# WoojuLee24/OA-DG

Hardware: AMD Instinct MI355X
Metric: images/sec training, Faster R-CNN R50-FPN + OA-DG, 1024x2048 (higher is better)
Workload: dtype bf16

## Files before the change

include/oadg_hip.h:

```cpp
#ifndef OADG_HIP_H
#define OADG_HIP_H

#include <stddef.h>
#include <stdint.h>

#ifdef __cplusplus
extern "C" {
#endif

size_t oadg_supcon_workspace_bytes(int B, int D);
int oadg_supcon_fwd(const float* feats, const int64_t* labels, int B, int D, int n_labels, int ori_size,
                    int rp_size, float temper, int min_samples, float loss_weight, void* workspace,
                    size_t workspace_bytes, float* out_loss, void* stream);
int oadg_supcon_bwd(const int64_t* labels, int B, int D, int n_labels, int ori_size, int rp_size,
                    float temper, float loss_weight, const float* grad_out, void* workspace,
                    size_t workspace_bytes, float* dfeats, void* stream);
int oadg_supcon_status(const void* workspace_host_copy);

size_t oadg_cls_loss_workspace_bytes(void);
int oadg_ce_jsd_fwd(const float* logits, const int64_t* labels, const float* weights, long R, int C,
                    int mode, float avg_factor, float loss_weight, float lambda_jsd, void* workspace,
                    size_t workspace_bytes, float* out3, void* stream);
int oadg_ce_jsd_bwd(const float* logits, const int64_t* labels, const float* weights, long R, int C,
                    int mode, float avg_factor, float loss_weight, float lambda_jsd, const float* grad_out,
                    float* dlogits, void* stream);

int oadg_roi_align_fwd(const void* const* feats_host, const int* heights_host, const int* widths_host,
                       const float* scales_host, int levels, int N, int C, int dtype, float finest_scale,
                       const float* rois, int K, int PH, int PW, int sampling_ratio, int aligned,
                       void* out, const int* order, void* stream);
int oadg_roi_align_bwd(float* const* dfeats_host, const int* heights_host, const int* widths_host,
                       const float* scales_host, int levels, int N, int C, int dtype, float finest_scale,
                       const float* rois, int K, int PH, int PW, int sampling_ratio, int aligned,
                       const void* grad_out, const int* order, void* stream);
int oadg_roi_order_keys(const float* rois, int K, int n_img, int levels, float finest_scale, long long* keys,
                        void* stream);
int oadg_roi_order(const float* rois, int K, int n_img, int levels, float finest_scale, int* order, int* range,
                   void* stream);
int oadg_roi_align_bwd_tiles(void* const* dmaps, const int* heights, const int* widths, const float* scales,
                             int levels, int N, int C, float finest_scale, const float* rois, int K, int PH, int PW,
                             int sampling_ratio, int aligned, const void* grad_out, const int* order, const int* range,
                             void* tile_boxes, void* stream);

typedef struct oadg_rpn_loss_level {
    const void* y;
    void* gy;
    long sN, sC, sH, sW;
    int H, W, Cy;
    long first, pix0;
} oadg_rpn_loss_level;
size_t oadg_rpn_loss_workspace_bytes(void);
int oadg_rpn_loss_fwd(const oadg_rpn_loss_level* levels, int n_levels, int B, int A, long At, int dtype,
                      const int64_t* labels, const float* label_weights, const float* bbox_targets,
                      const float* bbox_weights, float avg_factor, float w_cls, float lambda_jsd, float w_box,
                      void* workspace, size_t workspace_bytes, float* out4, void* stream);
int oadg_rpn_loss_bwd(const oadg_rpn_loss_level* levels, int n_levels, int B, int A, long At, int dtype,
                      const int64_t* labels, const float* label_weights, const float* bbox_targets,
                      const float* bbox_weights, float avg_factor, float w_cls, float lambda_jsd, float w_box,
                      const float* grad_cls, const float* grad_box, void* stream);

#define OADG_RPN_MAX_LEVELS 8
typedef struct oadg_rpn_level {
    const void* deltas;
    long sN, sC, sH, sW;
    const float* anchors;
    const float* scores;
    const long long* index;
    int H, W, A, k, dtype, first;
} oadg_rpn_level;
int oadg_rpn_decode(const oadg_rpn_level* levels, int n_levels, int n_img, const float* means4, const float* stds4,
                    float max_ratio, const float* lim, int clip, float min_size, float* props, float* scores,
                    unsigned char* valid, void* stream);
int oadg_rpn_order(const oadg_rpn_level* levels, int n_levels, int n_img, const float* props, const float* scores,
                   const unsigned char* valid, float* boxes_sorted, int* order, int* counts, float* max_coord,
                   void* stream);
// ... 212 lines not shown

int oadg_conv2d_nhwc_bf16_scatter(const void* x, const void* w, const float* bias, const void* residual, void* y,
                                  const void* zeros16, int N, int H, int W, int C, int K, int R, int S, int pad, int dil,
                                  int relu, int out_h, int out_w, int OH, int OW, int osh, int osw, int oph, int opw,
                                  const void* mask, float* colsum_part, const void* mask_bits, void* stream);
int oadg_conv2d_dgrad_s2_nhwc_bf16(const void* dy, const void* wt, const void* residual, void* dx, const void* zeros16,
                                   int N, int Ho, int Wo, int K, int C, int R, int H, int W, const void* mask,
                                   float* colsum_part, const void* mask_bits, void* stream);

int oadg_prep_conv_weights(const float* w, const float* gamma, const float* beta, const float* mean,
                           const float* var, float eps, const float* bias_in, int K, int C, int R, int S, void* wf,
                           void* wt, float* bias, float* scale, int w_krsc, int wt_mode, void* stream);
typedef struct oadg_prep_desc {
    const float *w, *gamma, *beta, *mean, *var, *bias_in;
    void *wf, *wt;
    float *bias, *scale;
    float eps;
    int K, C, R, S, w_krsc, wt_mode, first_block;
} oadg_prep_desc;
int oadg_prep_conv_weights_multi_blocks(int K, int C, int R, int S);
int oadg_prep_conv_weights_multi(const oadg_prep_desc* descs, int n_layers, int total_blocks, void* stream);
int oadg_prep_conv_weights_bwd(const void* gwf, const float* gbias, const float* w, const float* scale,
                               const float* mean, const float* var, float eps, int K, int C, int R, int S, float* dw,
                               float* dgamma, int w_krsc, void* stream);

int oadg_conv1x1_n16_fwd(const void* x, const void* w16, const float* bias16, void* y, long M, int C, void* stream);
long oadg_conv1x1_n16_dgrad_rows(long M);
int oadg_conv1x1_n16_dgrad(const void* dy, const void* wt, void* dx, const void* mask_bits, float* colsum_part, long M, int C,
                           void* stream);
long oadg_conv1x1_n16_wgrad_splits(long M);
long oadg_conv1x1_n16_wgrad_rows(long M);
int oadg_conv1x1_n16_wgrad(const void* x, const void* dy, float* part, float* bias_part, const void* zeros16, long M, int C,
                           void* stream);

int oadg_stem_conv7x7s2_nhwc_bf16(const void* x, const void* wp, void* y, int N, int H, int W, void* stream);

int oadg_bias_relu_maxpool_nhwc_bf16(const void* x, const float* bias, void* out, int N, int H, int W, int C,
                                     void* stream);

size_t oadg_relu_bias_bwd_workspace_bytes(long M, int K);
int oadg_relu_bias_bwd(const void* dy, int dy_is_f32, const void* y, void* g, float* dbias, void* workspace,
                       size_t workspace_bytes, long M, int K, void* stream);

int oadg_fpn_topdown_fwd(const void* lat, const void* top, void* out, int N, int H, int W, int Ht, int Wt, int C,
                         void* stream);
int oadg_fpn_topdown_bwd(const void* g, void* dtop, int N, int H, int W, int Ht, int Wt, int C, void* stream);

size_t oadg_max_iou_assign_workspace_bytes(int B, int Gmax);
int oadg_max_iou_assign(const float* boxes, long box_stride, const unsigned char* valid, const float* gts,
                        const int* gt_counts, const int64_t* gt_labels, int B, int N, int Gmax, float pos_iou_thr,
                        float neg_iou_lo, float neg_iou_hi, float min_pos_iou, int match_low_quality,
                        void* workspace, size_t workspace_bytes, int64_t* gt_inds, float* max_overlaps,
                        int64_t* labels, int* counts, void* stream);

typedef struct oadg_select_job {
    const void* gt_inds;
    long n;
    int mode;
    int k;
    int all;
    int rank_off;
    long out_off;
} oadg_select_job;
size_t oadg_sample_select_workspace_bytes(int jobs, long max_n);
int oadg_sample_select(const oadg_select_job* jobs_dev, int jobs, long max_n, int max_k, const int* ranks_dev,
                       int64_t* out, void* workspace, size_t workspace_bytes, void* stream);
// ... 104 lines not shown
```

oa-dg_amd/_lib.py:

```python
import ctypes
import os
from ctypes import (POINTER, Structure, c_char_p, c_double, c_float, c_int, c_int32, c_int64, c_long, c_longlong, c_size_t,
                    c_uint16, c_void_p)

import numpy as np

_HERE = os.path.dirname(os.path.abspath(__file__))
LIB_PATH = os.environ.get('OADG_HIP_LIB') or os.path.join(_HERE, 'csrc', 'liboadg_hip.so')
_lib = None

vp, ci, cf, cl, cs, cd = c_void_p, c_int, c_float, c_long, c_size_t, c_double


class RpnLevel(Structure):
    _fields_ = [('deltas', c_void_p), ('sN', c_long), ('sC', c_long), ('sH', c_long), ('sW', c_long), ('anchors', c_void_p),
                ('scores', c_void_p), ('index', c_void_p), ('H', c_int), ('W', c_int), ('A', c_int), ('k', c_int),
                ('dtype', c_int), ('first', c_int)]


class RpnLossLevel(Structure):
    _fields_ = [('y', c_void_p), ('gy', c_void_p), ('sN', c_long), ('sC', c_long), ('sH', c_long), ('sW', c_long),
                ('H', c_int), ('W', c_int), ('Cy', c_int), ('first', c_long), ('pix0', c_long)]


class RoiAssignImage(Structure):
    _fields_ = [('proposals', c_void_p), ('gt_bboxes', c_void_p), ('gt_labels', c_void_p), ('stride', c_int),
                ('num_gts', c_int)]


ROI_ASSIGN_MAX_IMAGES = 32


class RoiTargetEntry(Structure):
    _fields_ = [('bboxes', c_void_p), ('gt_bboxes', c_void_p), ('gt_inds', c_void_p), ('labels', c_void_p),
                ('pos_inds', c_void_p), ('neg_inds', c_void_p), ('npos', c_int), ('nneg', c_int), ('stride', c_int),
                ('batch', c_int)]


ROI_TARGET_MAX_ENTRIES = 32


class RoiSampleImage(Structure):
    _fields_ = [('gt_inds', c_void_p), ('n', c_int)]


ROI_SAMPLE_MAX_IMAGES = 8
RPN_MAX_LEVELS = 8
PARSE_LOSSES_MAX = 32


class RegionOp(Structure):
    _fields_ = [('kind', c_int), ('param', c_int), ('image', c_void_p), ('minv', c_double * 6)]


OP_COPY, OP_LUT_AUTOCONTRAST, OP_LUT_EQUALIZE, OP_POSTERIZE, OP_SOLARIZE, OP_IMAGE, OP_BG_WARP, OP_WARP_NEG = range(8)
# ... 25 lines not shown
        _f(ci, 'K C R S w_krsc wt_mode first_block')


class SelectJob(Structure):
    _fields_ = [('gt_inds', vp), ('n', cl)] + _f(ci, 'mode k all rank_off') + [('out_off', cl)]


class SgdTensor(Structure):
    _fields_ = _f(vp, 'param grad momentum') + _f(c_longlong, 'numel first_block') + _f(ci, 'first_step pad')


class MixTarget(Structure):
    _fields_ = [('fg_index', ci), ('rect', ci * 4), ('m_oa', cf)]


class BboxStep(Structure):
    _fields_ = [('minv', cd * 6), ('rect', ci * 4), ('row', ci), ('pad_', ci), ('scratch_off', c_longlong)]


class BboxChain(Structure):
    _fields_ = _f(vp, 'img steps_dev tile_prefix_dev level_first_host tile_prefix_host My Mx scratch') + \
        _f(ci, 'H W n_levels pad_')


class JpegDesc(Structure):
    _fields_ = _f(c_int32, 'height width ncomp hmax vmax mcux mcuy reserved') + _f(c_int32 * 4, 'h v bw bh cw ch') + \
        [('off', c_int64 * 4), ('qt', c_uint16 * 64 * 4)]


COLSUM_JOB, WGRAD_JOB, PREP_BWD_JOB, PREP_DESC, SELECT_JOB, SGD_TENSOR, MIX_TARGET, BBOX_STEP, BBOX_CHAIN = (
    np.dtype(c) for c in (ColsumJob, WgradJob, PrepBwdJob, PrepDesc, SelectJob, SgdTensor, MixTarget, BboxStep, BboxChain))

STRUCTS = {
    'oadg_rpn_level': RpnLevel, 'oadg_rpn_loss_level': RpnLossLevel, 'oadg_roi_assign_image': RoiAssignImage,
    'oadg_roi_target_entry': RoiTargetEntry, 'oadg_roi_sample_image': RoiSampleImage, 'oadg_region_op': RegionOp,
    'oadg_colsum_job': ColsumJob, 'oadg_wgrad_job': WgradJob, 'oadg_prep_bwd_job': PrepBwdJob, 'oadg_prep_desc': PrepDesc,
    'oadg_select_job': SelectJob, 'oadg_sgd_tensor': SgdTensor, 'oadg_mix_target': MixTarget, 'oadg_bbox_step': BboxStep,
    'oadg_bbox_chain': BboxChain, 'oadg_jpeg_desc': JpegDesc,
}

SIGNATURES = {
    'oadg_supcon_workspace_bytes': (cs, [ci, ci]),
    'oadg_supcon_fwd': (ci, [vp, vp, ci, ci, ci, ci, ci, cf, ci, cf, vp, cs, vp, vp]),
    'oadg_supcon_bwd': (ci, [vp, ci, ci, ci, ci, ci, cf, cf, vp, vp, cs, vp, vp]),
    'oadg_supcon_status': (ci, [vp]),
    'oadg_cls_loss_workspace_bytes': (cs, []),
    'oadg_ce_jsd_fwd': (ci, [vp, vp, vp, cl, ci, ci, cf, cf, cf, vp, cs, vp, vp]),
    'oadg_ce_jsd_bwd': (ci, [vp, vp, vp, cl, ci, ci, cf, cf, cf, vp, vp, vp]),
    'oadg_roi_align_fwd': (ci, [POINTER(vp), POINTER(ci), POINTER(ci), POINTER(cf), ci, ci, ci, ci, cf,
                                vp, ci, ci, ci, ci, ci, vp, vp, vp]),
    'oadg_roi_align_bwd': (ci, [POINTER(vp), POINTER(ci), POINTER(ci), POINTER(cf), ci, ci, ci, ci, cf,
                                vp, ci, ci, ci, ci, ci, vp, vp, vp]),
    'oadg_roi_order_keys': (ci, [vp, ci, ci, ci, cf, vp, vp]),
    'oadg_roi_order': (ci, [vp, ci, ci, ci, cf, vp, vp, vp]),
    'oadg_roi_align_bwd_tiles': (ci, [POINTER(vp), POINTER(ci), POINTER(ci), POINTER(cf), ci, ci, ci, cf, vp, ci, ci, ci,
                                      ci, ci, vp, vp, vp, vp, vp]),
    'oadg_rpn_loss_workspace_bytes': (cs, []),
    'oadg_rpn_loss_fwd': (ci, [vp, ci, ci, ci, cl, ci, vp, vp, vp, vp, cf, cf, cf, cf, vp, cs, vp, vp]),
    'oadg_rpn_loss_bwd': (ci, [vp, ci, ci, ci, cl, ci, vp, vp, vp, vp, cf, cf, cf, cf, vp, vp, vp]),
    'oadg_rpn_decode': (ci, [vp, ci, ci, vp, vp, cf, vp, ci, cf, vp, vp, vp, vp]),
    'oadg_rpn_order': (ci, [vp, ci, ci, vp, vp, vp, vp, vp, vp, vp, vp]),
    'oadg_rpn_gather': (ci, [ci, ci, ci, vp, vp, vp, vp, vp, vp, vp]),
    'oadg_rpn_topk_workspace_bytes': (cs, [POINTER(ci), ci, ci, ci]),
    'oadg_rpn_topk': (ci, [POINTER(vp), POINTER(cl), POINTER(ci), ci, ci, ci, ci, POINTER(vp), POINTER(vp), vp, cs, vp]),
    'oadg_nms_workspace_bytes': (cs, [ci, ci]),
    'oadg_nms_batched': (ci, [vp, vp, ci, ci, cf, ci, vp, cs, vp, vp, vp]),
    'oadg_resize_bilinear_u8': (ci, [vp, ci, ci, ci, vp, ci, ci, vp]),
    'oadg_flip_u8': (ci, [vp, ci, ci, ci, vp, ci, vp]),
    'oadg_conv2d_nhwc_bf16': (ci, [vp, vp, vp, vp, vp, vp] + [ci] * 11 + [vp]),
    'oadg_conv2d_auto_variant': (ci, [ci] * 10),
    'oadg_conv2d_nhwc_bf16_ex': (ci, [vp, vp, vp, vp, vp, vp] + [ci] * 12 + [vp, vp, vp, vp, vp]),
    'oadg_conv2d_pixel_tiles': (cl, [ci] * 11),
    'oadg_colsum_reduce': (ci, [vp, cl, ci, vp, vp]),
    'oadg_conv2d_nhwc_bf16_variant': (ci, [vp, vp, vp, vp, vp, vp] + [ci] * 12 + [vp]),
    'oadg_conv2d_wgrad_workspace_bytes': (cs, [ci] * 7),
    'oadg_conv2d_wgrad_variant': (ci, [ci] * 7),
    'oadg_conv2d_wgrad_nhwc_bf16': (ci, [vp, vp, vp, vp, vp, cs] + [ci] * 10 + [vp]),
    'oadg_conv2d_wgrad_parts_nhwc_bf16': (ci, [vp, vp, vp, vp, cs] + [ci] * 10 + [POINTER(ci), vp]),
    'oadg_prep_conv_weights_bwd_parts': (ci, [vp, ci, vp, vp, vp, vp, vp, cf, ci, ci, ci, ci, vp, vp, ci, vp]),
    'oadg_prep_conv_weights': (ci, [vp, vp, vp, vp, vp, cf, vp, ci, ci, ci, ci, vp, vp, vp, vp, ci, ci, vp]),
    'oadg_prep_conv_weights_multi': (ci, [vp, ci, ci, vp]),
    'oadg_prep_conv_weights_multi_blocks': (ci, [ci, ci, ci, ci]),
    'oadg_conv2d_nhwc_bf16_scatter': (ci, [vp, vp, vp, vp, vp, vp] + [ci] * 18 + [vp, vp, vp, vp]),
    'oadg_conv2d_dgrad_s2_nhwc_bf16': (ci, [vp, vp, vp, vp, vp, ci, ci, ci, ci, ci, ci, ci, ci, vp, vp, vp, vp]),
    'oadg_prep_conv_weights_bwd': (ci, [vp, vp, vp, vp, vp, vp, cf, ci, ci, ci, ci, vp, vp, ci, vp]),
    'oadg_relu_bias_bwd_workspace_bytes': (ctypes.c_size_t, [cl, ci]),
    'oadg_relu_bias_bwd': (ci, [vp, ci, vp, vp, vp, vp, ctypes.c_size_t, cl, ci, vp]),
    'oadg_stem_conv7x7s2_nhwc_bf16': (ci, [vp, vp, vp, ci, ci, ci, vp]),
    'oadg_bias_relu_maxpool_nhwc_bf16': (ci, [vp, vp, vp, ci, ci, ci, ci, vp]),
    'oadg_fpn_topdown_fwd': (ci, [vp, vp, vp, ci, ci, ci, ci, ci, ci, vp]),
    'oadg_fpn_topdown_bwd': (ci, [vp, vp, ci, ci, ci, ci, ci, ci, vp]),
    'oadg_max_iou_assign_workspace_bytes': (ctypes.c_size_t, [ci, ci]),
    'oadg_max_iou_assign': (ci, [vp, cl, vp, vp, vp, vp, ci, ci, ci, cf, cf, cf, cf, ci, vp, ctypes.c_size_t, vp, vp, vp,
                                 vp, vp]),
    'oadg_sample_select_workspace_bytes': (ctypes.c_size_t, [ci, cl]),
    'oadg_sample_select': (ci, [vp, ci, cl, ci, vp, vp, vp, ctypes.c_size_t, vp]),
    'oadg_anchor_targets': (ci, [vp, vp, vp, vp, vp, vp, ci, ci, ci, ci, c_int64, cf, vp, vp, vp, vp, vp, vp, vp]),
    'oadg_colsum_reduce_multi': (ci, [vp, ci, ci, vp]),
    'oadg_conv1x1_n16_fwd': (ci, [vp, vp, vp, vp, cl, ci, vp]),
    'oadg_conv1x1_n16_dgrad_rows': (cl, [cl]),
    'oadg_conv1x1_n16_dgrad': (ci, [vp, vp, vp, vp, vp, cl, ci, vp]),
    'oadg_bottleneck_frozen_256': (ci, [vp, vp, vp, vp, vp, vp, vp, vp, ci, ci, ci, vp]),
    'oadg_bottleneck_frozen_first_64': (ci, [vp, vp, vp, vp, vp, vp, vp, vp, vp, vp, ci, ci, ci, vp]),
    'oadg_conv1x1_n16_wgrad_splits': (cl, [cl]),
    'oadg_conv1x1_n16_wgrad_rows': (cl, [cl]),
    'oadg_conv1x1_n16_wgrad': (ci, [vp, vp, vp, vp, vp, cl, ci, vp]),
    'oadg_conv2d_wgrad_multi_plan': (ctypes.c_long, [vp, ci, ci, vp]),
    'oadg_conv2d_wgrad_multi': (ci, [vp, ci, ci, vp, vp, vp]),
    'oadg_prep_conv_weights_bwd_parts_multi': (ci, [vp, ci, ci, ci, vp]),
    'oadg_sgd_blocks': (ctypes.c_longlong, [ctypes.c_longlong]),
    'oadg_sgd_step_multi': (ci, [vp, ci, ctypes.c_longlong, cf, cf, cf, vp]),
    'oadg_fc_weight_permute': (ci, [vp, vp, ci, ci, ci, ci, vp]),
    'oadg_parse_losses': (ci, [vp, vp, ci, ci, ctypes.c_uint, vp, vp, vp]),
    'oadg_roi_reg_acc_fwd': (ci, [vp, ci, vp, ci, vp, vp, vp, ci, ci, ci, ci, ci, cf, cf, cf, vp, vp]),
    'oadg_roi_reg_bwd': (ci, [vp, ci, vp, vp, vp, ci, ci, ci, ci, cf, cf, cf, vp, vp, vp]),
    'oadg_roi_assign_add_gt': (ci, [vp, ci, ci, ci, cf, cf, cf, cf, ci, vp, vp, vp, vp, vp, vp, vp, vp, vp, ctypes.c_size_t,
                                    vp, vp]),
    'oadg_roi_targets': (ci, [vp, ci, ci, c_int64, cf, vp, vp, vp, vp, vp, vp, vp, vp, vp]),
    'oadg_roi_targets_dev': (ci, [vp, ci, ci, ci, vp, c_int64, cf, vp, vp, vp, vp, vp, vp, vp, vp, vp]),
    'oadg_roi_sample_max_rows': (ci, []),
    'oadg_roi_sample_device': (ci, [vp, ci, ci, ci, cd, vp, vp, vp, vp, vp, vp]),
    'oadg_conv2d_f32': (ci, [vp, vp, vp, vp, vp, ci, ci, ci, ci, ci, ci, ci, ci, ci, ci, ci, ci, ci, vp]),
    'oadg_conv2d_wgrad_f32_splits': (ci, [ci, ci, ci, ci, ci, ci, ci]),
    'oadg_conv2d_wgrad_f32': (ci, [vp, vp, vp, vp, cs, ci, ci, ci, ci, ci, ci, ci, ci, ci, ci, vp]),
    'oadg_host_randperm_prefix': (ci, [vp, POINTER(ci), POINTER(ctypes.c_uint64), c_int64, c_int64, vp]),
    'oadg_np_random_bboxes': (ci, [vp, ci, ci, ci, vp, ci, cd, cd, cd, cd, ci, cd, cd, vp]),
    'oadg_oamix_box_profiles': (ci, [vp, vp, ci, ci, ci, ci, vp, vp, vp]),
    'oadg_oamix_fg_union': (ci, [vp, vp, ci, ci, ci, vp, vp, vp]),
    'oadg_oamix_fg_union_rects': (ci, [vp, vp, vp, ci, ci, ci, vp, vp, vp]),
    'oadg_oamix_saliency_workspace_bytes': (cs, [ci]),
    'oadg_oamix_saliency': (ci, [vp, ci, ci, vp, ci, ci, vp, vp, cs, vp]),
    'oadg_oamix_saliency_batch': (ci, [vp, ctypes.c_longlong, vp, ci, ci, vp, ci, ci, vp, vp, ctypes.c_size_t, vp]),
    'oadg_oamix_hist': (ci, [vp, cl, vp, vp]),
    'oadg_oamix_luts': (ci, [vp, vp, vp]),
    'oadg_oamix_gray_sum': (ci, [vp, cl, vp, vp]),
    'oadg_oamix_bbox_step': (ci, [vp, ci, ci, POINTER(cd), ci, ci, ci, ci, vp, vp, vp, vp]),
    'oadg_oamix_bbox_levels': (ci, [POINTER(ci), POINTER(cd), ci, ci, ci, POINTER(ci)]),
    'oadg_oamix_bbox_plan_bytes': (cs, [ci]),
    'oadg_oamix_bbox_plan': (ci, [ci, cd, vp, vp, ci, vp, ci, ci, ci, vp, cs, vp, vp, vp]),
# ... 72 lines not shown
```

oa-dg_amd/csrc/narrow_head.hip:

```cpp
#include "common.h"
#include "oadg_hip.h"

namespace {

typedef float f32x4n __attribute__((ext_vector_type(4)));
typedef short v4sn __attribute__((ext_vector_type(4)));
typedef __attribute__((address_space(3))) v4sn* lds_v4sn_ptr;
typedef __attribute__((address_space(3))) void* lds_ptr_n;
typedef const __attribute__((address_space(1))) void* gbl_ptr_n;

__device__ __forceinline__ void glds16n(const void* g, void* l) {
    __builtin_amdgcn_global_load_lds((gbl_ptr_n)g, (lds_ptr_n)l, 16, 0, 0);
}

#define ZERO8 (bf16x8{0, 0, 0, 0, 0, 0, 0, 0})

__device__ __forceinline__ int kofs(int ks, int fq) { return 64 * (ks >> 1) + 16 * fq + 8 * (ks & 1); }

template <int C>
__global__ __launch_bounds__(256) void n16_fwd_kernel(const unsigned short* __restrict__ x,
                                                      const unsigned short* __restrict__ w16,
                                                      const float* __restrict__ bias16, unsigned short* __restrict__ y,
                                                      long M) {
    constexpr int KS = C / 32;
// ... 286 lines not shown
    const long splits = n16_splits(M), nchunks = (M + NWP - 1) / NWP;
    const int cps = (int)((nchunks + splits - 1) / splits);
    const unsigned grid = (unsigned)((nchunks + cps - 1) / cps);
    if ((long)grid != splits && (long)grid > splits) return OADG_EARG;
    hipStream_t st = (hipStream_t)stream;
#define OADG_N16W(CC)                                                                                                     \
    do {                                                                                                                  \
        constexpr int LDS = 2 * (NWP * CC * 2 + NWP * 32);                                                                \
        static bool attr = false;                                                                                         \
        if (!attr) {                                                                                                      \
            hipError_t e = hipFuncSetAttribute((const void*)n16_wgrad_kernel<CC>,                                         \
                                               hipFuncAttributeMaxDynamicSharedMemorySize, LDS);                          \
            if (e != hipSuccess) return (int)e;                                                                           \
            attr = true;                                                                                                  \
        }                                                                                                                 \
        hipLaunchKernelGGL(n16_wgrad_kernel<CC>, dim3(grid), dim3(256), LDS, st, (const unsigned short*)x,                \
                           (const unsigned short*)dy, part, bias_part, (const unsigned short*)zeros16, M, cps);           \
    } while (0)
    if (C == 256) OADG_N16W(256);
    else if (C == 128) OADG_N16W(128);
    else return OADG_EARG;
#undef OADG_N16W
    OADG_LAUNCH_CHECK();
    return OADG_OK;
}

long oadg_conv1x1_n16_wgrad_rows(long M) {
    if (M < 1) return 0;
    const long splits = n16_splits(M), nchunks = (M + NWP - 1) / NWP;
    const long cps = (nchunks + splits - 1) / splits;
    return (nchunks + cps - 1) / cps;
}

}
```

oa-dg_amd/csrc/roi_align.hip:

```cpp
#include "common.h"
#include <stdlib.h>

#define OADG_MAX_LEVELS 8

namespace {

struct Pyramid {
    const void* feat[OADG_MAX_LEVELS];
    float* dfeat[OADG_MAX_LEVELS];
    int H[OADG_MAX_LEVELS];
    int W[OADG_MAX_LEVELS];
    float scale[OADG_MAX_LEVELS];
    int levels;
    int N;
    int C;
    float finest_scale;
    const int* order;
};

__device__ __forceinline__ int roi_level(const float* roi, const Pyramid& p) {
    if (p.levels == 1) return 0;
    const float s = sqrtf((roi[3] - roi[1]) * (roi[4] - roi[2]));
    float l = floorf(log2f(s / p.finest_scale + 1e-6f));
    l = fminf(fmaxf(l, 0.f), (float)(p.levels - 1));
// ... 393 lines not shown
constexpr int HB = 32;

struct TileTables {
    float wy[RB_MAXP][TILE], wx[RB_MAXP][TILE];
    int plo, phi, qlo, qhi;
};

__global__ void roi_tile_box_kernel(Pyramid p, const float* __restrict__ rois, int K, int PH, int PW, int sampling_ratio,
                                    int aligned, const int* __restrict__ order, int4* __restrict__ boxes) {
    const int i = blockIdx.x * blockDim.x + threadIdx.x;
    if (i >= K) return;
    const int k = order[i];
    const RoiGeom g = roi_geom(rois + (size_t)k * 5, p, PH, PW, sampling_ratio, aligned);
    const int H = p.H[g.lvl], W = p.W[g.lvl];
    const float rh = g.bin_h * PH, rw = g.bin_w * PW;
    float ylo = floorf(g.start_h) - 1.f, yhi = ceilf(g.start_h + rh) + 1.f;
    float xlo = floorf(g.start_w) - 1.f, xhi = ceilf(g.start_w + rw) + 1.f;
    int4 b;
    if (g.batch < 0 || g.batch >= p.N || !(yhi >= 0.f) || !(xhi >= 0.f) || !(ylo < (float)H) || !(xlo < (float)W)) {
        b = make_int4(1, 1, g.lvl, -1);
    } else {
        ylo = fmaxf(ylo, 0.f); xlo = fmaxf(xlo, 0.f);
        yhi = fminf(yhi, (float)(H - 1)); xhi = fminf(xhi, (float)(W - 1));
        const int ty0 = (int)ylo / TILE, ty1 = (int)yhi / TILE, tx0 = (int)xlo / TILE, tx1 = (int)xhi / TILE;
        b = make_int4(tx0 | (tx1 << 16), ty0 | (ty1 << 16), g.lvl, g.batch);
    }
    boxes[i] = b;
}

__device__ __forceinline__ float lane_f(float v, int l) {
    return __builtin_bit_cast(float, __builtin_amdgcn_readlane(__builtin_bit_cast(int, v), l));
}

__global__ __launch_bounds__(TB_THREADS, 4) void roi_align_bwd_tiles_kernel(Pyramid p, TileGrid tg, const float* __restrict__ rois,
                                                                         int PH, int PW, int sampling_ratio, int aligned,
                                                                         const unsigned short* __restrict__ gout,
                                                                         const int* __restrict__ order,
                                                                         const int* __restrict__ range,
                                                                         const int4* __restrict__ boxes, int tpw) {
    __shared__ TileTables tab[HB];
    __shared__ int hits[TB_THREADS * TPW];
    __shared__ int wcnt[TPW * 8], wbase[TPW * 8 + 1];
    const int tid = threadIdx.x, lane = tid & 63;
    const int wave = __builtin_amdgcn_readfirstlane(tid >> 6);
    const int chunk = wave & 3, xh = wave >> 2;
    int lvl = 0;
    while (lvl + 1 < p.levels && (int)blockIdx.x >= tg.first[lvl + 1]) ++lvl;
    const int H = p.H[lvl], W = p.W[lvl], C = p.C;
    const int txl = tg.tx[lvl];
    const int per_img = txl * tg.ty[lvl];
    const int wg_per_img = (per_img + tpw - 1) / tpw;
    const int local = blockIdx.x - tg.first[lvl];
    const int n = local / wg_per_img, t_first = (local - n * wg_per_img) * tpw;
    const int n_t = min(tpw, per_img - t_first);
    const int r0 = range[lvl * p.N + n], r1 = range[lvl * p.N + n + 1];
    const int bins = PH * PW;
    unsigned short* dst = reinterpret_cast<unsigned short*>(const_cast<void*>(p.feat[lvl])) + (size_t)n * H * W * C;
    const int cb = blockIdx.y * 256;
    const int cw = min(256, C - cb);
    const bool chan_ok = chunk * 64 + lane < cw;
    const unsigned short* gcol = gout + cb + chunk * 64 + lane;

    float acc[TILE][TILE / 2];
#pragma unroll
    for (int y = 0; y < TILE; ++y)
#pragma unroll
        for (int x = 0; x < TILE / 2; ++x) acc[y][x] = 0.f;
    int cur_t = 0;

    auto flush = [&](int tt) {
        const int t = t_first + tt;
        const int tyi = t / txl, txi = t - tyi * txl;
        const int y0 = tyi * TILE, x0 = txi * TILE;
#pragma unroll
        for (int y = 0; y < TILE; ++y)
#pragma unroll
            for (int x = 0; x < TILE / 2; ++x) {
                const int py = y0 + y, px = x0 + xh * 4 + x;
                if (py < H && px < W) dst[((size_t)py * W + px) * C + cb + chunk * 64 + lane] = f32_to_bf16(acc[y][x]);
                acc[y][x] = 0.f;
            }
    };
    auto load_block = [&](float (&v)[4][4], int kk, int pb, int qb) {
        const unsigned short* gk = gcol + (size_t)kk * bins * C;
#pragma unroll
        for (int i = 0; i < 4; ++i) {
            const int pr = min(pb + i, PH - 1) * PW;
#pragma unroll
            for (int j = 0; j < 4; ++j) v[i][j] = bf16_to_f32(gk[(size_t)(pr + min(qb + j, PW - 1)) * C]);
        }
    };
    auto process = [&](int nh) {
        for (int hb = 0; hb < nh; hb += HB) {
            __syncthreads();
            {
                const int hi_ = hb + (tid >> 4), sub = tid & 15;
                const bool rows = sub < 8;
                const int bin = sub & 7, nb = rows ? PH : PW;
                bool nz = false;
                if (hi_ < nh) {
                    TileTables& tb = tab[tid >> 4];
                    float* w = rows ? tb.wy[bin] : tb.wx[bin];
                    if (bin < nb) {
                        const int hv = hits[hi_];
                        const int t = t_first + (hv >> 24);
                        const int tyi = t / txl, txi = t - tyi * txl;
                        const RoiGeom g = roi_geom(rois + (size_t)(hv & 0xffffff) * 5, p, PH, PW, sampling_ratio, aligned);
                        if (rows) axis_tile_weights(g.start_h, g.bin_h, g.grid_h, bin, H, tyi * TILE, w);
                        else axis_tile_weights(g.start_w, g.bin_w, g.grid_w, bin, W, txi * TILE, w);
                        const float inv = rows ? 1.0f / g.count : 1.0f;
#pragma unroll
                        for (int j = 0; j < TILE; ++j) {
                            const float v = w[j];
                            nz = nz || v != 0.f;
// ... 99 lines not shown
            if ((mm[tt] >> lane) & 1ull)
                hits[wbase[tt * 8 + wave] + __popcll(mm[tt] & ((1ull << lane) - 1ull))] = myk | (tt << 24);
        process(wbase[64]);
    } else {
        for (int tt = 0; tt < n_t; ++tt) {
            const int t = t_first + tt;
            const int tyi = t / txl, txi = t - tyi * txl;
            for (int rb = r0; rb < r1; rb += TB_THREADS) {
                bool hit = false;
                int k = -1;
                if (rb + tid < r1) {
                    const int4 b = boxes[rb + tid];
                    hit = b.z == lvl && b.w == n && txi >= (b.x & 0xffff) && txi <= (b.x >> 16) &&
                          tyi >= (b.y & 0xffff) && tyi <= (b.y >> 16);
                    if (hit) k = order[rb + tid];
                }
                const unsigned long long m = __ballot(hit);
                __syncthreads();
                if (lane == 0) wcnt[wave] = __popcll(m);
                __syncthreads();
                int base = 0, nh = 0;
#pragma unroll
                for (int w2 = 0; w2 < TB_THREADS / 64; ++w2) {
                    if (w2 < wave) base += wcnt[w2];
                    nh += wcnt[w2];
                }
                if (hit) hits[base + __popcll(m & ((1ull << lane) - 1ull))] = k | (tt << 24);
                process(nh);
            }
        }
    }
    if (chan_ok)
        while (cur_t < n_t) { flush(cur_t); ++cur_t; }
}

__device__ __forceinline__ long long roi_order_key(const float* __restrict__ rois, int k, int n_img, int levels,
                                                   float finest_scale) {
    const float* r = rois + (size_t)k * 5;
    const float w = fmaxf(r[3] - r[1], 0.f), h = fmaxf(r[4] - r[2], 0.f);
    float l = floorf(log2f(sqrtf(w * h) / finest_scale + 1e-6f));
    l = fminf(fmaxf(l, 0.f), (float)(levels - 1));
    const int lvl = (int)l;
    const float cell = 64.f * (float)(1 << lvl);
    int qx = (int)((r[1] + r[3]) * 0.5f / cell), qy = (int)((r[2] + r[4]) * 0.5f / cell);
    qx = qx < 0 ? 0 : (qx > 1023 ? 1023 : qx);
    qy = qy < 0 ? 0 : (qy > 1023 ? 1023 : qy);
    int b = (int)r[0];
    b = b < 0 ? 0 : (b >= n_img ? n_img - 1 : b);
    return (((long long)lvl * n_img + b) * 1024 + qy) * 1024 + qx;
}

__global__ void roi_order_key_kernel(const float* __restrict__ rois, int K, int n_img, int levels, float finest_scale,
                                     long long* __restrict__ keys) {
    const int k = blockIdx.x * blockDim.x + threadIdx.x;
    if (k < K) keys[k] = roi_order_key(rois, k, n_img, levels, finest_scale);
}

__global__ __launch_bounds__(256) void roi_order_rank_kernel(const float* __restrict__ rois, int K, int n_img, int levels,
                                                             float finest_scale, int* __restrict__ order,
                                                             int* __restrict__ range) {
    extern __shared__ __attribute__((aligned(16))) unsigned long long rk_keys[];
    const int Kp = (K + 7) & ~7;
    for (int j = threadIdx.x; j < Kp; j += 256)
        rk_keys[j] = j < K ? ((unsigned long long)roi_order_key(rois, j, n_img, levels, finest_scale) << 16) | (unsigned)j
                           : ~0ull;
    __syncthreads();
// ... 75 lines not shown
}

int oadg_roi_order(const float* rois, int K, int n_img, int levels, float finest_scale, int* order, int* range,
                   void* stream) {
    if (!rois || !order || !range || K < 1 || K > 8192 || n_img < 1 || levels < 1 || levels > OADG_MAX_LEVELS) return OADG_EARG;
    hipLaunchKernelGGL(roi_order_rank_kernel, dim3((K + 255) / 256), dim3(256), (size_t)((K + 7) & ~7) * sizeof(unsigned long long),
                       (hipStream_t)stream, rois, K, n_img, levels, finest_scale, order, range);
    OADG_LAUNCH_CHECK();
    return OADG_OK;
}

int oadg_roi_align_bwd(float* const* dfeats, const int* heights, const int* widths, const float* scales,
                       int levels, int N, int C, int dtype, float finest_scale, const float* rois, int K,
                       int PH, int PW, int sampling_ratio, int aligned, const void* grad_out,
                       const int* order, void* stream) {
    if (!dfeats || !heights || !widths || !scales || !rois || !grad_out) return OADG_EARG;
    if (K < 0 || PH < 1 || PW < 1 || (dtype != 0 && dtype != 1)) return OADG_EARG;
    Pyramid p;
    const int rc = fill_pyramid(p, nullptr, dfeats, heights, widths, scales, levels, N, C, finest_scale);
    if (rc) return rc;
    p.order = order;
    if (K == 0) return OADG_OK;
    hipStream_t st = (hipStream_t)stream;
    if (dtype == 0)
        hipLaunchKernelGGL((roi_align_bwd_kernel<float>), dim3(K), dim3(256), 0, st, p, rois, K, PH, PW,
                           sampling_ratio, aligned, (const float*)grad_out);
    else
        hipLaunchKernelGGL((roi_align_bwd_kernel<unsigned short>), dim3(K), dim3(256), 0, st, p, rois, K,
                           PH, PW, sampling_ratio, aligned, (const unsigned short*)grad_out);
    OADG_LAUNCH_CHECK();
    return OADG_OK;
}

int oadg_roi_align_bwd_tiles(void* const* dmaps, const int* heights, const int* widths, const float* scales,
                             int levels, int N, int C, float finest_scale, const float* rois, int K, int PH, int PW,
                             int sampling_ratio, int aligned, const void* grad_out, const int* order, const int* range,
                             void* tile_boxes, void* stream) {
    if (!dmaps || !heights || !widths || !scales || !rois || !grad_out || !order || !range || !tile_boxes) return OADG_EARG;
    if (K < 0 || PH < 1 || PW < 1 || PH > RB_MAXP || PW > RB_MAXP) return OADG_EARG;
    Pyramid p;
    const int rc = fill_pyramid(p, (const void* const*)dmaps, nullptr, heights, widths, scales, levels, N, C, finest_scale);
    if (rc) return rc;
    TileGrid tg;
    const int nchunk = (C + 255) / 256;
    long tiles = 0;
    for (int l = 0; l < levels; ++l) tiles += (long)N * ((widths[l] + TILE - 1) / TILE) * ((heights[l] + TILE - 1) / TILE);
    int tpw = (int)(tiles * nchunk / 2048);
    tpw = tpw < 1 ? 1 : (tpw > TPW ? TPW : tpw);
    int total = 0;
    for (int l = 0; l < levels; ++l) {
        tg.first[l] = total;
        tg.tx[l] = (widths[l] + TILE - 1) / TILE;
        tg.ty[l] = (heights[l] + TILE - 1) / TILE;
        total += N * ((tg.tx[l] * tg.ty[l] + tpw - 1) / tpw);
    }
    tg.first[levels] = total;
    if (K > 0) {
        hipLaunchKernelGGL(roi_tile_box_kernel, dim3((K + 255) / 256), dim3(256), 0, (hipStream_t)stream, p, rois, K, PH, PW,
                           sampling_ratio, aligned, order, (int4*)tile_boxes);
        OADG_LAUNCH_CHECK();
    }
    hipLaunchKernelGGL(roi_align_bwd_tiles_kernel, dim3(total, nchunk), dim3(TB_THREADS), 0, (hipStream_t)stream, p, tg, rois, PH,
                       PW, sampling_ratio, aligned, (const unsigned short*)grad_out, order, range, (const int4*)tile_boxes, tpw);
    OADG_LAUNCH_CHECK();
    return OADG_OK;
}

}
```

Before: 146.2.

## Add fused RoIAlign-backward accumulate/colsum kernel and RPN branch backward entry point

Adds an accumulating variant of the tiled RoIAlign backward kernel. It adds an existing gradient base map into the scattered tile gradients and emits per-tile channel column sums for the downstream bias gradient, which avoids separate add and reduction passes. It also adds a combined RPN branch backward entry that runs the loss backward plus the 1x1 dgrad and wgrad per level in one host call. Python bindings are added, but the diff shows no caller, so the new paths may not run by default.

```diff
diff --git a/include/oadg_hip.h b/include/oadg_hip.h
--- a/include/oadg_hip.h
+++ b/include/oadg_hip.h
@@ -41,6 +41,11 @@
                              int levels, int N, int C, float finest_scale, const float* rois, int K, int PH, int PW,
                              int sampling_ratio, int aligned, const void* grad_out, const int* order, const int* range,
                              void* tile_boxes, void* stream);
+int oadg_roi_align_bwd_tiles_rows(const int* heights, const int* widths, int levels, int N, int C, long* rows_out);
+int oadg_roi_align_bwd_tiles_acc(void* const* dmaps, const void* const* bases, float* const* colsum_parts, const int* heights,
+                                 const int* widths, const float* scales, int levels, int N, int C, float finest_scale,
+                                 const float* rois, int K, int PH, int PW, int sampling_ratio, int aligned,
+                                 const void* grad_out, const int* order, const int* range, void* tile_boxes, void* stream);
 
 typedef struct oadg_rpn_loss_level {
     const void* y;
@@ -319,6 +324,20 @@
 long oadg_conv1x1_n16_wgrad_rows(long M);
 int oadg_conv1x1_n16_wgrad(const void* x, const void* dy, float* part, float* bias_part, const void* zeros16, long M, int C,
                            void* stream);
+typedef struct oadg_rpn_branch_level {
+    const void* x;
+    void* gx;
+    const void* mask_bits;
+    float* colsum_part;
+    float* wpart;
+    float* bpart;
+    long M;
+} oadg_rpn_branch_level;
+int oadg_rpn_branch_bwd(const oadg_rpn_loss_level* loss_levels, const oadg_rpn_branch_level* levels, int n_levels, int B, int A,
+                        long At, const int64_t* labels, const float* label_weights, const float* bbox_targets,
+                        const float* bbox_weights, float avg_factor, float w_cls, float lambda_jsd, float w_box,
+                        const float* grad_cls, const float* grad_box, const void* wt16, const void* zeros16, int C,
+                        void* stream);
 
 int oadg_stem_conv7x7s2_nhwc_bf16(const void* x, const void* wp, void* y, int N, int H, int W, void* stream);
 
diff --git a/oa-dg_amd/_lib.py b/oa-dg_amd/_lib.py
--- a/oa-dg_amd/_lib.py
+++ b/oa-dg_amd/_lib.py
@@ -21,6 +21,11 @@
 class RpnLossLevel(Structure):
     _fields_ = [('y', c_void_p), ('gy', c_void_p), ('sN', c_long), ('sC', c_long), ('sH', c_long), ('sW', c_long),
                 ('H', c_int), ('W', c_int), ('Cy', c_int), ('first', c_long), ('pix0', c_long)]
+
+
+class RpnBranchLevel(Structure):
+    _fields_ = [('x', c_void_p), ('gx', c_void_p), ('mask_bits', c_void_p), ('colsum_part', c_void_p), ('wpart', c_void_p),
+                ('bpart', c_void_p), ('M', c_long)]
 
 
 class RoiAssignImage(Structure):
@@ -112,7 +117,8 @@
     np.dtype(c) for c in (ColsumJob, WgradJob, PrepBwdJob, PrepDesc, SelectJob, SgdTensor, MixTarget, BboxStep, BboxChain))
 
 STRUCTS = {
-    'oadg_rpn_level': RpnLevel, 'oadg_rpn_loss_level': RpnLossLevel, 'oadg_roi_assign_image': RoiAssignImage,
+    'oadg_rpn_level': RpnLevel, 'oadg_rpn_loss_level': RpnLossLevel, 'oadg_rpn_branch_level': RpnBranchLevel,
+    'oadg_roi_assign_image': RoiAssignImage,
     'oadg_roi_target_entry': RoiTargetEntry, 'oadg_roi_sample_image': RoiSampleImage, 'oadg_region_op': RegionOp,
     'oadg_colsum_job': ColsumJob, 'oadg_wgrad_job': WgradJob, 'oadg_prep_bwd_job': PrepBwdJob, 'oadg_prep_desc': PrepDesc,
     'oadg_select_job': SelectJob, 'oadg_sgd_tensor': SgdTensor, 'oadg_mix_target': MixTarget, 'oadg_bbox_step': BboxStep,
@@ -135,6 +141,9 @@
     'oadg_roi_order': (ci, [vp, ci, ci, ci, cf, vp, vp, vp]),
     'oadg_roi_align_bwd_tiles': (ci, [POINTER(vp), POINTER(ci), POINTER(ci), POINTER(cf), ci, ci, ci, cf, vp, ci, ci, ci,
                                       ci, ci, vp, vp, vp, vp, vp]),
+    'oadg_roi_align_bwd_tiles_rows': (ci, [POINTER(ci), POINTER(ci), ci, ci, ci, POINTER(cl)]),
+    'oadg_roi_align_bwd_tiles_acc': (ci, [POINTER(vp), POINTER(vp), POINTER(vp), POINTER(ci), POINTER(ci), POINTER(cf), ci, ci,
+                                          ci, cf, vp, ci, ci, ci, ci, ci, vp, vp, vp, vp, vp]),
     'oadg_rpn_loss_workspace_bytes': (cs, []),
     'oadg_rpn_loss_fwd': (ci, [vp, ci, ci, ci, cl, ci, vp, vp, vp, vp, cf, cf, cf, cf, vp, cs, vp, vp]),
     'oadg_rpn_loss_bwd': (ci, [vp, ci, ci, ci, cl, ci, vp, vp, vp, vp, cf, cf, cf, cf, vp, vp, vp]),
@@ -185,6 +194,7 @@
     'oadg_conv1x1_n16_wgrad_splits': (cl, [cl]),
     'oadg_conv1x1_n16_wgrad_rows': (cl, [cl]),
     'oadg_conv1x1_n16_wgrad': (ci, [vp, vp, vp, vp, vp, cl, ci, vp]),
+    'oadg_rpn_branch_bwd': (ci, [vp, vp, ci, ci, ci, cl, vp, vp, vp, vp, cf, cf, cf, cf, vp, vp, vp, vp, ci, vp]),
     'oadg_conv2d_wgrad_multi_plan': (ctypes.c_long, [vp, ci, ci, vp]),
     'oadg_conv2d_wgrad_multi': (ci, [vp, ci, ci, vp, vp, vp]),
     'oadg_prep_conv_weights_bwd_parts_multi': (ci, [vp, ci, ci, ci, vp]),
diff --git a/oa-dg_amd/csrc/narrow_head.hip b/oa-dg_amd/csrc/narrow_head.hip
--- a/oa-dg_amd/csrc/narrow_head.hip
+++ b/oa-dg_amd/csrc/narrow_head.hip
@@ -342,4 +342,31 @@
     return (nchunks + cps - 1) / cps;
 }
 
-}
+int oadg_rpn_branch_bwd(const oadg_rpn_loss_level* loss_levels, const oadg_rpn_branch_level* levels, int n_levels, int B, int A,
+                        long At, const int64_t* labels, const float* label_weights, const float* bbox_targets,
+                        const float* bbox_weights, float avg_factor, float w_cls, float lambda_jsd, float w_box,
+                        const float* grad_cls, const float* grad_box, const void* wt16, const void* zeros16, int C,
+                        void* stream) {
+    if (!loss_levels || !levels || n_levels < 1 || n_levels > OADG_RPN_MAX_LEVELS || !wt16 || !zeros16) return OADG_EARG;
+    if (C != 128 && C != 256) return OADG_EARG;
+    for (int l = 0; l < n_levels; ++l) {
+        const oadg_rpn_loss_level& q = loss_levels[l];
+        const oadg_rpn_branch_level& v = levels[l];
+        if (!q.gy || q.Cy != 16 || v.M != (long)B * q.H * q.W || v.M < 1) return OADG_EARG;
+        if (!v.x || !v.gx || !v.wpart || !v.bpart) return OADG_EARG;
+    }
+    int rc = oadg_rpn_loss_bwd(loss_levels, n_levels, B, A, At, 1, labels, label_weights, bbox_targets, bbox_weights, avg_factor,
+                               w_cls, lambda_jsd, w_box, grad_cls, grad_box, stream);
+    if (rc) return rc;
+    for (int l = 0; l < n_levels; ++l) {
+        const oadg_rpn_branch_level& v = levels[l];
+        const void* dy = loss_levels[l].gy;
+        rc = oadg_conv1x1_n16_dgrad(dy, wt16, v.gx, v.mask_bits, v.colsum_part, v.M, C, stream);
+        if (rc) return rc;
+        rc = oadg_conv1x1_n16_wgrad(v.x, dy, v.wpart, v.bpart, zeros16, v.M, C, stream);
+        if (rc) return rc;
+    }
+    return OADG_OK;
+}
+
+}
diff --git a/oa-dg_amd/csrc/roi_align.hip b/oa-dg_amd/csrc/roi_align.hip
--- a/oa-dg_amd/csrc/roi_align.hip
+++ b/oa-dg_amd/csrc/roi_align.hip
@@ -449,12 +449,17 @@
     return __builtin_bit_cast(float, __builtin_amdgcn_readlane(__builtin_bit_cast(int, v), l));
 }
 
-__global__ __launch_bounds__(TB_THREADS, 4) void roi_align_bwd_tiles_kernel(Pyramid p, TileGrid tg, const float* __restrict__ rois,
-                                                                         int PH, int PW, int sampling_ratio, int aligned,
-                                                                         const unsigned short* __restrict__ gout,
-                                                                         const int* __restrict__ order,
-                                                                         const int* __restrict__ range,
-                                                                         const int4* __restrict__ boxes, int tpw) {
+struct TileAcc {
+    const unsigned short* base[OADG_MAX_LEVELS];
+    float* part[OADG_MAX_LEVELS];
+};
+
+template <bool ACC>
+__device__ __forceinline__ void roi_bwd_tiles_body(const Pyramid& p, const TileGrid& tg, const TileAcc& ta,
+                                                   const float* __restrict__ rois, int PH, int PW, int sampling_ratio,
+                                                   int aligned, const unsigned short* __restrict__ gout,
+                                                   const int* __restrict__ order, const int* __restrict__ range,
+                                                   const int4* __restrict__ boxes, int tpw) {
     __shared__ TileTables tab[HB];
     __shared__ int hits[TB_THREADS * TPW];
     __shared__ int wcnt[TPW * 8], wbase[TPW * 8 + 1];
@@ -484,19 +489,50 @@
 #pragma unroll
         for (int x = 0; x < TILE / 2; ++x) acc[y][x] = 0.f;
     int cur_t = 0;
+    const unsigned short* bsrc = nullptr;
+    float csum = 0.f;
+    if constexpr (ACC)
+        if (ta.base[lvl]) bsrc = ta.base[lvl] + (size_t)n * H * W * C;
 
     auto flush = [&](int tt) {
         const int t = t_first + tt;
         const int tyi = t / txl, txi = t - tyi * txl;
         const int y0 = tyi * TILE, x0 = txi * TILE;
-#pragma unroll
-        for (int y = 0; y < TILE; ++y)
-#pragma unroll
-            for (int x = 0; x < TILE / 2; ++x) {
-                const int py = y0 + y, px = x0 + xh * 4 + x;
-                if (py < H && px < W) dst[((size_t)py * W + px) * C + cb + chunk * 64 + lane] = f32_to_bf16(acc[y][x]);
-                acc[y][x] = 0.f;
-            }
+        if constexpr (ACC) {
+#pragma unroll
+            for (int y2 = 0; y2 < TILE; y2 += 2) {
+                float bv[2][TILE / 2];
+#pragma unroll
+                for (int yy = 0; yy < 2; ++yy)
+#pragma unroll
+                    for (int x = 0; x < TILE / 2; ++x) {
+                        const int py = y0 + y2 + yy, px = x0 + xh * 4 + x;
+                        bv[yy][x] = (bsrc && py < H && px < W)
+                                        ? bf16_to_f32(bsrc[((size_t)py * W + px) * C + cb + chunk * 64 + lane]) : 0.f;
+                    }
+#pragma unroll
+                for (int yy = 0; yy < 2; ++yy)
+#pragma unroll
+                    for (int x = 0; x < TILE / 2; ++x) {
+                        const int y = y2 + yy, py = y0 + y, px = x0 + xh * 4 + x;
+                        if (py < H && px < W) {
+                            const unsigned short r = f32_to_bf16(bsrc ? acc[y][x] + bv[yy][x] : acc[y][x]);
+                            dst[((size_t)py * W + px) * C + cb + chunk * 64 + lane] = r;
+                            csum += bf16_to_f32(r);
+                        }
+                        acc[y][x] = 0.f;
+                    }
+            }
+        } else {
+#pragma unroll
+            for (int y = 0; y < TILE; ++y)
+#pragma unroll
+                for (int x = 0; x < TILE / 2; ++x) {
+                    const int py = y0 + y, px = x0 + xh * 4 + x;
+                    if (py < H && px < W) dst[((size_t)py * W + px) * C + cb + chunk * 64 + lane] = f32_to_bf16(acc[y][x]);
+                    acc[y][x] = 0.f;
+                }
+        }
     };
     auto load_block = [&](float (&v)[4][4], int kk, int pb, int qb) {
         const unsigned short* gk = gcol + (size_t)kk * bins * C;
@@ -662,6 +698,34 @@
     }
     if (chan_ok)
         while (cur_t < n_t) { flush(cur_t); ++cur_t; }
+    if constexpr (ACC) {
+        float* part = ta.part[lvl];
+        if (part) {
+            __shared__ float right[256];
+            if (xh == 1) right[chunk * 64 + lane] = csum;
+            __syncthreads();
+            if (xh == 0 && chan_ok) part[(size_t)local * C + cb + chunk * 64 + lane] = csum + right[chunk * 64 + lane];
+        }
+    }
+}
+
+__global__ __launch_bounds__(TB_THREADS, 4) void roi_align_bwd_tiles_kernel(Pyramid p, TileGrid tg, const float* __restrict__ rois,
+                                                                         int PH, int PW, int sampling_ratio, int aligned,
+                                                                         const unsigned short* __restrict__ gout,
+                                                                         const int* __restrict__ order,
+                                                                         const int* __restrict__ range,
+                                                                         const int4* __restrict__ boxes, int tpw) {
+    roi_bwd_tiles_body<false>(p, tg, TileAcc{}, rois, PH, PW, sampling_ratio, aligned, gout, order, range, boxes, tpw);
+}
+
+__global__ __launch_bounds__(TB_THREADS, 4) void roi_align_bwd_tiles_acc_kernel(Pyramid p, TileGrid tg, TileAcc ta,
+                                                                             const float* __restrict__ rois, int PH, int PW,
+                                                                             int sampling_ratio, int aligned,
+                                                                             const unsigned short* __restrict__ gout,
+                                                                             const int* __restrict__ order,
+                                                                             const int* __restrict__ range,
+                                                                             const int4* __restrict__ boxes, int tpw) {
+    roi_bwd_tiles_body<true>(p, tg, ta, rois, PH, PW, sampling_ratio, aligned, gout, order, range, boxes, tpw);
 }
 
 __device__ __forceinline__ long long roi_order_key(const float* __restrict__ rois, int k, int n_img, int levels,
@@ -803,16 +867,7 @@
     return OADG_OK;
 }
 
-int oadg_roi_align_bwd_tiles(void* const* dmaps, const int* heights, const int* widths, const float* scales,
-                             int levels, int N, int C, float finest_scale, const float* rois, int K, int PH, int PW,
-                             int sampling_ratio, int aligned, const void* grad_out, const int* order, const int* range,
-                             void* tile_boxes, void* stream) {
-    if (!dmaps || !heights || !widths || !scales || !rois || !grad_out || !order || !range || !tile_boxes) return OADG_EARG;
-    if (K < 0 || PH < 1 || PW < 1 || PH > RB_MAXP || PW > RB_MAXP) return OADG_EARG;
-    Pyramid p;
-    const int rc = fill_pyramid(p, (const void* const*)dmaps, nullptr, heights, widths, scales, levels, N, C, finest_scale);
-    if (rc) return rc;
-    TileGrid tg;
+static int tile_grid(TileGrid& tg, const int* heights, const int* widths, int levels, int N, int C, int* tpw_out) {
     const int nchunk = (C + 255) / 256;
     long tiles = 0;
     for (int l = 0; l < levels; ++l) tiles += (long)N * ((widths[l] + TILE - 1) / TILE) * ((heights[l] + TILE - 1) / TILE);
@@ -826,15 +881,71 @@
         total += N * ((tg.tx[l] * tg.ty[l] + tpw - 1) / tpw);
     }
     tg.first[levels] = total;
+    *tpw_out = tpw;
+    return total;
+}
+
+static int roi_bwd_tiles_launch(void* const* dmaps, const void* const* bases, float* const* colsum_parts, bool acc,
+                                const int* heights, const int* widths, const float* scales, int levels, int N, int C,
+                                float finest_scale, const float* rois, int K, int PH, int PW, int sampling_ratio, int aligned,
+                                const void* grad_out, const int* order, const int* range, void* tile_boxes, void* stream) {
+    if (!dmaps || !heights || !widths || !scales || !rois || !grad_out || !order || !range || !tile_boxes) return OADG_EARG;
+    if (K < 0 || PH < 1 || PW < 1 || PH > RB_MAXP || PW > RB_MAXP) return OADG_EARG;
+    Pyramid p;
+    const int rc = fill_pyramid(p, (const void* const*)dmaps, nullptr, heights, widths, scales, levels, N, C, finest_scale);
+    if (rc) return rc;
+    TileGrid tg;
+    int tpw;
+    const int total = tile_grid(tg, heights, widths, levels, N, C, &tpw);
+    const int nchunk = (C + 255) / 256;
     if (K > 0) {
         hipLaunchKernelGGL(roi_tile_box_kernel, dim3((K + 255) / 256), dim3(256), 0, (hipStream_t)stream, p, rois, K, PH, PW,
                            sampling_ratio, aligned, order, (int4*)tile_boxes);
         OADG_LAUNCH_CHECK();
     }
-    hipLaunchKernelGGL(roi_align_bwd_tiles_kernel, dim3(total, nchunk), dim3(TB_THREADS), 0, (hipStream_t)stream, p, tg, rois, PH,
-                       PW, sampling_ratio, aligned, (const unsigned short*)grad_out, order, range, (const int4*)tile_boxes, tpw);
+    if (acc) {
+        TileAcc ta;
+        for (int l = 0; l < OADG_MAX_LEVELS; ++l) {
+            ta.base[l] = (l < levels && bases) ? (const unsigned short*)bases[l] : nullptr;
+            ta.part[l] = (l < levels && colsum_parts) ? colsum_parts[l] : nullptr;
+        }
+        hipLaunchKernelGGL(roi_align_bwd_tiles_acc_kernel, dim3(total, nchunk), dim3(TB_THREADS), 0, (hipStream_t)stream, p, tg, ta,
+                           rois, PH, PW, sampling_ratio, aligned, (const unsigned short*)grad_out, order, range,
+                           (const int4*)tile_boxes, tpw);
+    } else {
+        hipLaunchKernelGGL(roi_align_bwd_tiles_kernel, dim3(total, nchunk), dim3(TB_THREADS), 0, (hipStream_t)stream, p, tg, rois,
+                           PH, PW, sampling_ratio, aligned, (const unsigned short*)grad_out, order, range,
+                           (const int4*)tile_boxes, tpw);
+    }
     OADG_LAUNCH_CHECK();
     return OADG_OK;
 }
 
-}
+int oadg_roi_align_bwd_tiles(void* const* dmaps, const int* heights, const int* widths, const float* scales,
+                             int levels, int N, int C, float finest_scale, const float* rois, int K, int PH, int PW,
+                             int sampling_ratio, int aligned, const void* grad_out, const int* order, const int* range,
+                             void* tile_boxes, void* stream) {
+    return roi_bwd_tiles_launch(dmaps, nullptr, nullptr, false, heights, widths, scales, levels, N, C, finest_scale, rois, K,
+                                PH, PW, sampling_ratio, aligned, grad_out, order, range, tile_boxes, stream);
+}
+
+int oadg_roi_align_bwd_tiles_rows(const int* heights, const int* widths, int levels, int N, int C, long* rows_out) {
+    if (!heights || !widths || !rows_out || levels < 1 || levels > OADG_MAX_LEVELS || N < 1 || C < 4) return OADG_EARG;
+    for (int l = 0; l < levels; ++l)
+        if (heights[l] < 1 || widths[l] < 1) return OADG_EARG;
+    TileGrid tg;
+    int tpw;
+    tile_grid(tg, heights, widths, levels, N, C, &tpw);
+    for (int l = 0; l < levels; ++l) rows_out[l] = tg.first[l + 1] - tg.first[l];
+    return OADG_OK;
+}
+
+int oadg_roi_align_bwd_tiles_acc(void* const* dmaps, const void* const* bases, float* const* colsum_parts, const int* heights,
+                                 const int* widths, const float* scales, int levels, int N, int C, float finest_scale,
+                                 const float* rois, int K, int PH, int PW, int sampling_ratio, int aligned,
+                                 const void* grad_out, const int* order, const int* range, void* tile_boxes, void* stream) {
+    return roi_bwd_tiles_launch(dmaps, bases, colsum_parts, true, heights, widths, scales, levels, N, C, finest_scale, rois, K,
+                                PH, PW, sampling_ratio, aligned, grad_out, order, range, tile_boxes, stream);
+}
+
+}
```

Result: slower. 144.5 (-1.2%).
